# tayloraswift/jpeg

Hardware: AMD Instinct MI355X
Metric: Mpixels/s decode (IDCT+dequant+upsample+YCbCr->RGB); % HBM roofline (higher is better)
Workload: dtype f32; 1 GPU; C3: one 8192x8192 ycc8 4:2:0 image per GPU per step, fused Spectral->RGB8 decode (ring of 4 distinct images); sampling=4:2:0, output=RGB8, coefficients=distribution N (SURVEY 8d), seeded, quanta=CompressionLevel luminance/chrominance(1.0), parallelism=independent images x1 (weak scaling), no data-path collective

## Files before the change

include/jpeg_amd.h:

```cpp
#ifndef JPEG_AMD_H
#define JPEG_AMD_H

#include <stddef.h>
#include <stdint.h>

#ifdef __cplusplus
extern "C" {
#endif

#define JPEG_AMD_VERSION 100
#define JPEG_AMD_MAX_PLANES 4

typedef enum jpeg_amd_status {
    JPEG_AMD_OK      = 0,
    JPEG_AMD_EINVAL  = -1,
    JPEG_AMD_ENOMEM  = -2,
    JPEG_AMD_EHIP    = -3,
    JPEG_AMD_ENODEV  = -4,
    JPEG_AMD_ENOSUP  = -5
} jpeg_amd_status;

typedef struct jpeg_amd_ctx jpeg_amd_ctx;

typedef struct jpeg_amd_layout {
// ... 9 lines not shown
} jpeg_amd_layout;

typedef enum jpeg_amd_color {
    JPEG_AMD_COLOR_YCC8 = 0,
    JPEG_AMD_COLOR_RGB8 = 1
} jpeg_amd_color;

int         jpeg_amd_version(void);
const char *jpeg_amd_strerror(int status);
int         jpeg_amd_device_count(int *count);
#define JPEG_AMD_CTX_OWN_STREAM 1
int         jpeg_amd_ctx_create(int device, void *stream, int flags, jpeg_amd_ctx **ctx);
int         jpeg_amd_ctx_destroy(jpeg_amd_ctx *ctx);
int         jpeg_amd_ctx_synchronize(jpeg_amd_ctx *ctx);
int         jpeg_amd_last_hip_error(const jpeg_amd_ctx *ctx);
int         jpeg_amd_layout_units(jpeg_amd_layout *layout);

int jpeg_amd_malloc(jpeg_amd_ctx *ctx, size_t bytes, void **d_ptr);
int jpeg_amd_free(jpeg_amd_ctx *ctx, void *d_ptr);
int jpeg_amd_memcpy_h2d(jpeg_amd_ctx *ctx, void *d_dst, const void *h_src, size_t bytes);
int jpeg_amd_memcpy_d2h(jpeg_amd_ctx *ctx, void *h_dst, const void *d_src, size_t bytes);
int jpeg_amd_timer_begin(jpeg_amd_ctx *ctx);
int jpeg_amd_timer_end(jpeg_amd_ctx *ctx, float *elapsed_ms);


int jpeg_amd_idct_plane(jpeg_amd_ctx *ctx, const int16_t *d_coef, int units_x, int units_y,
                        const uint16_t h_quanta_zigzag[64], int precision,
                        uint16_t *d_plane);

int jpeg_amd_spectral_idct(jpeg_amd_ctx *ctx, const jpeg_amd_layout *layout,
// ... 257 lines not shown
```

include/jpeg_amd.hpp:

```cpp
#pragma once

#include <cstdint>
#include <algorithm>
#include <array>
#include <map>
#include <memory>
#include <stdexcept>
#include <string>
#include <utility>
#include <vector>

#include "jpeg_amd.h"

namespace jpeg_amd {

struct error : std::runtime_error {
    int status;
    error(int s, const std::string &what) : std::runtime_error(what + ": " + jpeg_amd_strerror(s)), status(s) {}
};
inline void check(int status, const char *what)
{
    if (status != JPEG_AMD_OK) throw error(status, what);
}

class context {
  public:
    explicit context(int device = 0, void *stream = nullptr, bool own_stream = true)
    {
        check(jpeg_amd_ctx_create(device, stream, own_stream ? JPEG_AMD_CTX_OWN_STREAM : 0, &ctx_), "jpeg_amd_ctx_create");
    }
    ~context() { jpeg_amd_ctx_destroy(ctx_); }
    context(const context &) = delete;
    context &operator=(const context &) = delete;
    jpeg_amd_ctx *handle() const { return ctx_; }
    void synchronize() const { check(jpeg_amd_ctx_synchronize(ctx_), "jpeg_amd_ctx_synchronize"); }

  private:
    jpeg_amd_ctx *ctx_ = nullptr;
};

template <class T>
class device_array {
  public:
    device_array() = default;
    device_array(const context &c, size_t n) : ctx_(&c), n_(n)
    {
        void *p = nullptr;
        check(jpeg_amd_malloc(c.handle(), n * sizeof(T), &p), "jpeg_amd_malloc");
        p_ = static_cast<T *>(p);
    }
// ... 360 lines not shown
```

jpeg_amd/_lib.py:

```python
from __future__ import annotations

import ctypes as C
import os

HERE = os.path.dirname(os.path.abspath(__file__))
LIB_PATH = os.environ.get("JPEG_AMD_LIBRARY") or os.path.join(HERE, "libjpeg_amd.so")
MAX_PLANES = 4

OK, EINVAL, ENOMEM, EHIP, ENODEV, ENOSUP = 0, -1, -2, -3, -4, -5
COLOR_YCC8, COLOR_RGB8 = 0, 1
CTX_OWN_STREAM = 1


class JpegAmdError(RuntimeError):
    def __init__(self, status: int, what: str, hip: int = 0):
        self.status, self.hip = status, hip
        msg = lib().jpeg_amd_strerror(status).decode()
        super().__init__(f"{what}: {msg} (status {status}" + (f", hipError {hip})" if hip else ")"))


class Layout(C.Structure):
    _fields_ = [
        ("width", C.c_int32), ("height", C.c_int32), ("precision", C.c_int32),
        ("nplanes", C.c_int32), ("scale_x", C.c_int32), ("scale_y", C.c_int32),
# ... 4 lines not shown


_p = C.c_void_p
_pp = C.POINTER(C.c_void_p)
_szp = C.POINTER(C.c_size_t)
_L = C.POINTER(Layout)

SIGNATURES = {
    "jpeg_amd_version": (C.c_int, []),
    "jpeg_amd_strerror": (C.c_char_p, [C.c_int]),
    "jpeg_amd_device_count": (C.c_int, [C.POINTER(C.c_int)]),
    "jpeg_amd_ctx_create": (C.c_int, [C.c_int, _p, C.c_int, _pp]),
    "jpeg_amd_ctx_destroy": (C.c_int, [_p]),
    "jpeg_amd_ctx_synchronize": (C.c_int, [_p]),
    "jpeg_amd_last_hip_error": (C.c_int, [_p]),
    "jpeg_amd_layout_units": (C.c_int, [_L]),
    "jpeg_amd_malloc": (C.c_int, [_p, C.c_size_t, _pp]),
    "jpeg_amd_free": (C.c_int, [_p, _p]),
    "jpeg_amd_memcpy_h2d": (C.c_int, [_p, _p, _p, C.c_size_t]),
    "jpeg_amd_memcpy_d2h": (C.c_int, [_p, _p, _p, C.c_size_t]),
    "jpeg_amd_timer_begin": (C.c_int, [_p]),
    "jpeg_amd_timer_end": (C.c_int, [_p, C.POINTER(C.c_float)]),
    "jpeg_amd_idct_plane": (C.c_int, [_p, _p, C.c_int, C.c_int, _p, C.c_int, _p]),
    "jpeg_amd_spectral_idct": (C.c_int, [_p, _L, _pp, _p, C.c_int, _pp]),
    "jpeg_amd_planar_interleaved": (C.c_int, [_p, _L, _pp, C.c_int, _p]),
    "jpeg_amd_rectangular_unpack": (C.c_int, [_p, _p, C.c_size_t, C.c_int, C.c_int, _p]),
    "jpeg_amd_decode_batch": (C.c_int, [_p, _L, C.c_int, _pp, _szp, _p, C.c_size_t, C.c_int,
                                        C.c_int, C.c_int, _p, C.c_size_t]),
    "jpeg_amd_decode": (C.c_int, [_p, _L, _pp, _p, C.c_int, C.c_int, C.c_int, _p]),
    "jpeg_amd_spectral_rectangular_batch": (C.c_int, [_p, _L, C.c_int, _pp, _szp, _p, C.c_size_t, C.c_int, C.c_int, _p, C.c_size_t]),
# ... 138 lines not shown
```

jpeg_amd/api.py:

```python
from __future__ import annotations

import ctypes as C
from dataclasses import dataclass
from typing import Dict, List, Optional, Sequence, Tuple

import numpy as np

from . import _lib

MAX_PLANES = _lib.MAX_PLANES


class YCbCr:
    code = _lib.COLOR_YCC8


class RGB:
    code = _lib.COLOR_RGB8


def _torch():
    import torch
    return torch

# ... 8 lines not shown
        self.device = int(device)
        self.torch_device = torch.device("cuda", self.device)
        if stream is None:
            stream = torch.cuda.current_stream(self.torch_device).cuda_stream
        self._h = C.c_void_p()
        flags = _lib.CTX_OWN_STREAM if own_stream else 0
        _lib.check(_lib.lib().jpeg_amd_ctx_create(self.device, C.c_void_p(stream), flags,
                                                 C.byref(self._h)), "jpeg_amd_ctx_create")

    @property
    def handle(self):
        return self._h

    def synchronize(self):
        _lib.check(_lib.lib().jpeg_amd_ctx_synchronize(self._h), "synchronize", self._h)

    def timer_begin(self):
        _lib.check(_lib.lib().jpeg_amd_timer_begin(self._h), "timer_begin", self._h)

    def timer_end(self) -> float:
        ms = C.c_float()
        _lib.check(_lib.lib().jpeg_amd_timer_end(self._h, C.byref(ms)), "timer_end", self._h)
        return ms.value

    def empty(self, n: int, dtype):
        torch = _torch()
        return torch.empty(max(int(n), 0), dtype=dtype, device=self.torch_device)

    def upload(self, a: np.ndarray):
        torch = _torch()
# ... 700 lines not shown
```

jpeg_amd/csrc/capi.hip:

```cpp
#pragma clang fp contract(off)

#include <hip/hip_runtime.h>

#include <cstdio>
#include <cstdlib>
#include <cstring>
#include <new>
#include <algorithm>
#include <atomic>
#include <memory>
#include <chrono>
#include <system_error>
#include <thread>
#include <vector>

#include "interleave.hpp"
#include "kernels.hpp"
#include "transform.hpp"
#include "worker_pool.hpp"

using namespace jpeg_amd;

struct jpeg_amd_ctx {
    int device = 0;
    hipStream_t stream = nullptr;
    bool own_stream = false;
    hipEvent_t ev_begin = nullptr, ev_end = nullptr;
    void *scratch = nullptr;
    size_t scratch_bytes = 0;
    uint16_t *d_qstage = nullptr;
    uint32_t *d_walk = nullptr;
    int32_t *d_flag = nullptr;
    void *d_region = nullptr;
    size_t region_bytes = 0;
    int qslot = 0;
    int last_hip = 0;
    void *file_pinned[2] = {nullptr, nullptr};
    void *file_device = nullptr;
    size_t file_pinned_bytes = 0, file_device_bytes = 0;
    hipEvent_t file_done[2] = {nullptr, nullptr};
    hipEvent_t file_decoded[2] = {nullptr, nullptr};
    hipEvent_t file_fetched[2] = {nullptr, nullptr};
    hipStream_t file_d2h = nullptr;
    std::unique_ptr<WorkerPool> workers, copiers;
    std::vector<std::vector<uint32_t>> records;
};
// ... 380 lines not shown
    if (ctx->ev_end) (void)hipEventDestroy(ctx->ev_end);
    if (ctx->own_stream && ctx->stream) (void)hipStreamDestroy(ctx->stream);
    delete ctx;
    return JPEG_AMD_OK;
}

int jpeg_amd_ctx_synchronize(jpeg_amd_ctx *ctx)
{
    JA_TRY(bind(ctx));
    JA_HIP(ctx, hipStreamSynchronize(ctx->stream));
    return JPEG_AMD_OK;
}

int jpeg_amd_last_hip_error(const jpeg_amd_ctx *ctx) { return ctx ? ctx->last_hip : 0; }

int jpeg_amd_layout_units(jpeg_amd_layout *L)
{
    if (!L || L->nplanes < 1 || L->nplanes > JPEG_AMD_MAX_PLANES || L->scale_x < 1 ||
        L->scale_y < 1 || L->width <= 0 || L->height <= 0)
        return JPEG_AMD_EINVAL;
    for (int p = 0; p < L->nplanes; ++p) {
        if (L->factor_x[p] < 1 || L->factor_y[p] < 1) return JPEG_AMD_EINVAL;
        L->units_x[p] = units_of(L->width * L->factor_x[p], 8 * L->scale_x);
        L->units_y[p] = units_of(L->height * L->factor_y[p], 8 * L->scale_y);
    }
    return JPEG_AMD_OK;
}


int jpeg_amd_malloc(jpeg_amd_ctx *ctx, size_t bytes, void **d_ptr)
// ... 126 lines not shown
                          const uint16_t *d_quanta, size_t quanta_stride, int ntables,
                          int cosited, jpeg_amd_color color, uint8_t *d_pixels,
                          size_t pixel_stride)
{
    JA_TRY(bind(ctx));
    JA_TRY(check_layout(L, ntables));
    JA_TRY(check_planes_cover_image(L));
    JA_TRY(check_batch8(L, n_images, color));
    if (n_images == 0) return JPEG_AMD_OK;
    if (!d_coef || !coef_stride || !d_quanta || !d_pixels) return JPEG_AMD_EINVAL;
    PlaneSet cs;
    JA_TRY(plane_set(L, d_coef, coef_stride, true, &cs));
    const QuantaRef q{d_quanta, quanta_stride};
    const bool rgb = color == JPEG_AMD_COLOR_RGB8;
    if (fused_decode_supported(*L, cosited != 0)) {
        JA_HIP(ctx, launch_fused_decode(ctx->stream, n_images, *L, cs, q, rgb, ctx->d_walk, d_pixels, pixel_stride));
        return JPEG_AMD_OK;
    }
    return staged_decode(ctx, L, n_images, cs, q, cosited != 0, true, rgb ? PixelKind::RGB8 : PixelKind::YCC8, d_pixels, pixel_stride);
}

int jpeg_amd_decode(jpeg_amd_ctx *ctx, const jpeg_amd_layout *L, const int16_t *const d_coef[],
                    const uint16_t *h_quanta, int ntables, int cosited, jpeg_amd_color color,
                    uint8_t *d_pixels)
{
    JA_TRY(bind(ctx));
    JA_TRY(check_layout(L, ntables));
    const uint16_t *d_q = nullptr;
    JA_TRY(stage_quanta(ctx, h_quanta, ntables, &d_q));
    const size_t zero[JPEG_AMD_MAX_PLANES] = {0, 0, 0, 0};
    return jpeg_amd_decode_batch(ctx, L, 1, d_coef, zero, d_q, 0, ntables, cosited, color,
// ... 1333 lines not shown
```

jpeg_amd/csrc/kernels.hpp:

```cpp
#pragma once

#include <hip/hip_runtime.h>
#include <stddef.h>
#include <stdint.h>

#include "../../include/jpeg_amd.h"

namespace jpeg_amd {

typedef uint32_t u32x4_t __attribute__((ext_vector_type(4)));
__device__ __forceinline__ void store_nt16(void *p, const uint4 &v)
{
    __builtin_nontemporal_store(u32x4_t{v.x, v.y, v.z, v.w}, reinterpret_cast<u32x4_t *>(p));
}

struct PlaneSet {
    const void *ptr[JPEG_AMD_MAX_PLANES];
    size_t      stride[JPEG_AMD_MAX_PLANES];
};
struct PlaneSetMut {
    void  *ptr[JPEG_AMD_MAX_PLANES];
    size_t stride[JPEG_AMD_MAX_PLANES];
};

// ... 19 lines not shown
hipError_t launch_planar_to_pixels(hipStream_t stream, int n_images,
                                   const jpeg_amd_layout &layout, const PlaneSet &planes,
                                   bool planes_u8, bool cosited, PixelKind kind,
                                   void *d_out, size_t out_stride_bytes);

bool       generic_encode_supported(const jpeg_amd_layout &layout);
hipError_t launch_generic_encode(hipStream_t stream, int n_images, const jpeg_amd_layout &layout, const uint16_t *d_rect,
                                 size_t rect_stride, QuantaRef q, const PlaneSetMut &coef);

hipError_t launch_unpack(hipStream_t stream, const uint16_t *d_rect, size_t npixels,
                         int nplanes, jpeg_amd_color color, uint8_t *d_pixels);

bool       fused_decode_supported(const jpeg_amd_layout &layout, bool cosited);
hipError_t launch_fused_decode(hipStream_t stream, int n_images, const jpeg_amd_layout &layout,
                               const PlaneSet &coef, QuantaRef q, bool rgb, uint32_t *d_walk_counters,
                               uint8_t *d_pixels, size_t pixel_stride);

bool       quad_decode_supported(const jpeg_amd_layout &layout);
hipError_t launch_quad_decode(hipStream_t stream, int n_images, const jpeg_amd_layout &layout,
                              const PlaneSet &coef, QuantaRef q, bool rgb, uint32_t *d_walk_counters,
                              uint8_t *d_pixels, size_t pixel_stride);

bool       generic_fused_supported(const jpeg_amd_layout &layout);
hipError_t launch_generic_fused(hipStream_t stream, int n_images, const jpeg_amd_layout &layout, const PlaneSet &coef,
                                QuantaRef q, bool cosited, uint32_t *d_walk_counter, uint16_t *d_rect, size_t rect_stride);

uint32_t   region_tiles(const jpeg_amd_region &region);
hipError_t launch_region_decode(hipStream_t stream, int n_images, const jpeg_amd_layout &layout, const PlaneSet &coef, QuantaRef q,
                                bool rgb, const uint32_t *d_tiles, const int32_t *d_regions, uint32_t nwg,
                                uint8_t *d_pixels, size_t pixel_stride);
hipError_t launch_region_crop(hipStream_t stream, int n_images, const uint8_t *d_full, size_t full_stride, int width,
                              const int32_t *d_regions, size_t max_bytes, uint8_t *d_pixels, size_t pixel_stride);

hipError_t launch_scaled_decode(hipStream_t stream, int n_images, const jpeg_amd_layout &layout, int n, int width, int height,
                                const PlaneSet &coef, QuantaRef q, bool rgb, uint8_t *d_pixels, size_t pixel_stride);
hipError_t launch_idct_scaled_plane(hipStream_t stream, int n_images, const int16_t *d_coef, size_t coef_stride, QuantaRef q,
// ... 24 lines not shown
```

jpeg_amd/csrc/kernels_fused.hip:

```cpp
#pragma clang fp contract(off)

#include "dct.hpp"
#include "fused_common.hpp"
#include "kernels.hpp"
#include "upsample.hpp"

#include <algorithm>
#include <cstdlib>

namespace jpeg_amd {

namespace {


struct LumaArgs {
    const int16_t *coef;
    size_t coef_stride;
    const int16_t *ccoef[2];
    size_t ccoef_stride[2];
    int cqi[2];
    const uint16_t *quanta;
    size_t quanta_stride;
    int qi;
    int ux, uy;
// ... 547 lines not shown
    for (int p = 0; p < L.nplanes; ++p) {
        if (L.units_x[p] != units(L.width * L.factor_x[p], 8 * L.scale_x)) return false;
        if (L.units_y[p] != units(L.height * L.factor_y[p], 8 * L.scale_y)) return false;
    }
    if (L.nplanes == 1) return true;
    if (L.nplanes != 3 || cosited) return false;
    if (L.factor_x[0] != L.scale_x || L.factor_y[0] != L.scale_y) return false;
    if (L.scale_x > 2 || L.scale_y > 2) return false;
    for (int p = 1; p < 3; ++p)
        if (L.factor_x[p] != 1 || L.factor_y[p] != 1) return false;
    return true;
}

hipError_t launch_fused_decode(hipStream_t stream, int n_images, const jpeg_amd_layout &L,
                               const PlaneSet &coef, QuantaRef q, bool rgb, uint32_t *d_walk_counters,
                               uint8_t *d_pixels, size_t pixel_stride)
{
    const bool chroma = L.nplanes == 3;
    if (chroma && L.scale_x == 2 && L.scale_y == 2)
        return launch_quad_decode(stream, n_images, L, coef, q, rgb, d_walk_counters, d_pixels, pixel_stride);
    LumaArgs la{};
    if (chroma) {
        for (int i = 0; i < 2; ++i) {
            la.ccoef[i] = static_cast<const int16_t *>(coef.ptr[1 + i]);
            la.ccoef_stride[i] = coef.stride[1 + i];
            la.cqi[i] = L.qi[1 + i];
        }
        la.pw_c = 8 * L.units_x[1]; la.ph_c = 8 * L.units_y[1];
    }
    la.coef = static_cast<const int16_t *>(coef.ptr[0]);
    la.coef_stride = coef.stride[0];
    la.quanta = q.d_quanta; la.quanta_stride = q.image_stride; la.qi = L.qi[0];
    la.ux = L.units_x[0]; la.uy = L.units_y[0];
    la.W = L.width; la.H = L.height;
    la.out = d_pixels; la.out_stride = pixel_stride;
// ... 28 lines not shown
```

jpeg_amd/csrc/kernels_quad.hip:

```cpp
#pragma clang fp contract(off)

#include "dct.hpp"
#include "fused_common.hpp"
#include "kernels.hpp"
#include "upsample.hpp"

#include <algorithm>
#include <cstdlib>

namespace jpeg_amd {

namespace {

JA_PHASE_STORAGE

struct QuadArgs {
    const int16_t *coef[3];
    size_t coef_stride[3];
    const uint16_t *quanta;
    size_t quanta_stride;
    int qi[3];
    int ux, uy;
    int uxc, uyc;
    int W, H;
    uint8_t *out;
    size_t out_stride;
    int tiles_x;
    int sx0;
    uint32_t *tickets;
    int stacks_per_image;
    int nstacks;
};

#ifndef JA_QUAD_WAVES
#define JA_QUAD_WAVES 3
#endif
template <int BX> struct QuadShape {
    static constexpr int BY = 64 / BX;
    static constexpr int QS = kThreads / 64;
};

template <int MODE, int BX, bool FAST, bool DYN>
__global__ __launch_bounds__(kThreads, JA_QUAD_WAVES) void k_quad420(QuadArgs a)
{
    constexpr int BY = QuadShape<BX>::BY, QS = QuadShape<BX>::QS;
    constexpr int NW = kThreads / 64;
    static_assert(QS == 4 && NW == 4, "the roles below are dealt to four waves");
    constexpr int CW = BX * 4, CR = BY * 4;
    constexpr int CBW = BX / 2, CBR = BY / 2;
    constexpr int PITCH = CW / 4 + 2;
    constexpr int QROWS = QS * CR + 2;
    constexpr int PLANE = QROWS * PITCH;
    constexpr int SEG_DW = BX * 6;
    constexpr int CPS = SEG_DW / 4;
    constexpr int NHROW = 4 * CBW, NSIDE = 4 * (QS * CBR + 2);
    constexpr int NDMA_C = 8;

#ifdef JA_X_LDSHACK
    __shared__ __attribute__((aligned(16))) uint32_t coefbuf[NW / 2][64 * 32];
// ... 26 lines not shown
        uint32_t rem, col;
        img = (int)fd_spi.div((uint32_t)q, rem);
        syi = QS * (int)fd_tx.div(rem, col) + qp;
        sxi = (int)col + a.sx0;
    };
    const int strips_y = (a.uy + BY - 1) / BY;
#ifdef JA_X_ROLEROT
    auto role_of = [&](int t) -> int { return (qp + t) & 3; };
#else
    auto role_of = [&](int t) -> int { return (qp + 2 * (t & 1)) & 3; };
#endif

    auto lane_chunk = [&](int lane) -> uint32_t {
        const uint32_t l3 = lane >> 3;
        return l3 * 128 + (((lane & 7) ^ (l3 >> 1)) << 4);
    };
    auto sgpr = [](uint32_t v) -> uint32_t { asm volatile("" : "+s"(v)); return v; };
    auto dma_luma = [&](int img, int syi, int sxi, int lane) {
        const uint32_t ve = lane_chunk(lane);
        const uint32_t ux = sgpr((uint32_t)a.ux);
        const uint32_t row0 = (uint32_t)(BY * syi), rows = (uint32_t)min(BY, a.uy - BY * syi);
        const char *base = reinterpret_cast<const char *>(a.coef[0] + img * a.coef_stride[0]) + ((uint64_t)(row0 * ux) << 7);
        const i32x4_t srd = make_srd(base, (rows * ux) << 7);
#pragma unroll
        for (int r = 0; r < BY; ++r)
            lds_dma16_brun<BX / 8, true>(srd, ((uint32_t)r * ux + (uint32_t)(sxi * BX)) << 7, ve, ve ^ 64u, coef_lds + r * (BX * 128));
    };
    auto dma_chroma = [&](int img, int syi, int sxi, int lane, int role) {
        const int top = syi - qp;
        const uint32_t uxc = sgpr((uint32_t)a.uxc);
// ... 24 lines not shown
            return;
        }
#pragma unroll
        for (int i = 0; i < NDMA_C; ++i) {
            if (8 * i >= NSIDE) break;
            const int b = 8 * i + (lane >> 3);
            const int pl = (b >> 1) & 1, row = min(max(CBR * top - 1 + (b >> 2), 0), a.uyc - 1);
            const int bx = (b & 1) ? CBW * sxi + CBW : CBW * sxi - 1;
            const int16_t *cbase = a.coef[1 + pl] + img * a.coef_stride[1 + pl];
            const uint32_t blk = (bx >= 0 && bx < a.uxc) ? (uint32_t)row * a.uxc + bx : 0u;
            const int c = (lane & 7) ^ ((b >> 1) & 7);
            lds_dma16_keep(reinterpret_cast<const char *>(cbase) + ((size_t)blk * 128 + 16 * c), coef_lds + 1024 * i);
        }
    };

#ifdef JA_X_STAGGER
    for (int d = (int)(blockIdx.x / 256u) * (JA_X_STAGGER); d > 0; d -= 64 * 100) __builtin_amdgcn_s_sleep(100);
#endif
    if ((int)blockIdx.x >= a.nstacks) return;
    constexpr bool dyn = DYN;
    int cur = (int)blockIdx.x;
    const int last_round = a.nstacks - (int)gridDim.x, second_last_round = a.nstacks - 2 * (int)gridDim.x;
    int c_img, c_syi, c_sxi;
    locate(cur, c_img, c_syi, c_sxi);
    dma_chroma(c_img, c_syi, c_sxi, lane0, role_of(0));
    int img_of_table = -1;
    int stores_behind_dma = 0;
    JA_PHASE_DECL

    for (int trip = 0;; ++trip) {
        int lane = lane0;
        asm volatile("" : "+v"(lane));
        const int lbx = lane & (BX - 1), seg = (int)((unsigned)lane / BX);
        const int img = c_img, syi = c_syi, sxi = c_sxi;
        const bool phantom = syi >= strips_y;

        const int table_id = a.quanta_stride == 0 ? 0 : img;
        if (table_id != img_of_table) {
            const int qk = lane & 7, qh = lane >> 3;
#pragma unroll
            for (int p = 0; p < 3; ++p)
                sqw[qp][p][8 * qk + qh] = modulate_entry(qk, qh, 0.125f, a.quanta[img * a.quanta_stride + 64 * a.qi[p] + zigzag_of(qk, qh)]);
            img_of_table = table_id;
        }

        if (stores_behind_dma == 16) asm volatile("s_waitcnt vmcnt(16)" ::: "memory");
        else asm volatile("s_waitcnt vmcnt(0)" ::: "memory");
        JA_PHASE(0)
        __builtin_amdgcn_s_setprio(3);
        uint32_t ticket = 0;
        if (dyn && qp == 0 && lane0 == 0) ticket = __hip_atomic_fetch_add(a.tickets, 1u, __ATOMIC_RELAXED, __HIP_MEMORY_SCOPE_AGENT);
        uint32_t w[32];
        auto read_block = [&]() {
            const uint4 *cw = reinterpret_cast<const uint4 *>(coef_w) + 8 * lane;
            const int sw = (lane >> 1) & 7;
#pragma unroll
            for (int i = 0; i < 8; ++i) {
                const uint4 v = cw[i ^ sw];
                w[4 * i + 0] = v.x; w[4 * i + 1] = v.y; w[4 * i + 2] = v.z; w[4 * i + 3] = v.w;
            }
        };
        read_block();
        const uint32_t done_seen = lds_peek(done);
        asm volatile("s_waitcnt lgkmcnt(0)" ::: "memory");
        if (!phantom) dma_luma(img, syi, sxi, lane);
        __builtin_amdgcn_sched_barrier(0);
        JA_PHASE(1)

        const int top = syi - qp;
        const bool stack_above = top > 0, stack_below = CBR * (top + QS) < a.uyc;
        const bool has_left = sxi > 0, has_right = CBW * sxi + CBW < a.uxc;
        const int first_bad = (a.uxc << 1) - sxi * (CW / 4) + 1;
        auto fix_columns = [&](uint32_t *row) {
            if (!has_left) row[0] = (row[1] & 0xffu) * 0x01010101u;
            if (first_bad < PITCH) {
                const uint32_t last = (row[first_bad - 1] >> 24) * 0x01010101u;
                for (int c = first_bad; c < PITCH; ++c) row[c] = last;
            }
        };
        {
// ... 61 lines not shown
#pragma unroll
                        for (int y = 0; y < 8; ++y) col[(1 + 8 * (rowi - 1) + y) * PITCH] = e[y];
                    }
                }
            }
        }
        lds_arrive(ready);
        JA_PHASE(4)
        if (cur < second_last_round) __builtin_amdgcn_s_setprio(2);
        else if (cur < last_round) __builtin_amdgcn_s_setprio(1);
        else __builtin_amdgcn_s_setprio(0);
        bool more = false;
        auto take = [&](int next) {
            more = next < a.nstacks;
            if (more) {
                int n_img, n_syi, n_sxi;
                locate(next, n_img, n_syi, n_sxi); c_img = n_img; c_syi = n_syi; c_sxi = n_sxi;
                dma_chroma(n_img, n_syi, n_sxi, lane, role_of(trip + 1));
                cur = next;
            }
        };
        auto drawn = [&]() -> int {
            lds_wait_ge(pub, (uint32_t)(trip + 1));
            return __builtin_amdgcn_readfirstlane((int)*(volatile uint32_t *)&next_slot[trip & 1]);
        };
        if (phantom) {
            if (dyn) take(drawn());
            else take(cur + (int)gridDim.x);
            lds_arrive(done);
            stores_behind_dma = 0;
            if (!more) break;
            continue;
        }
// ... 57 lines not shown
        auto finish = [&](float v) -> float {
            return __builtin_fmaf(v, 0.0625f, kMagic - 32768.0f - (MODE == 1 ? 128.0f : 0.0f)) - kMagic;
        };
        float hw[2][3][8];
        uint32_t rawn[2][3];
#pragma unroll
        for (int pl = 0; pl < 2; ++pl) {
            uint32_t r0[3], r1[3];
            hraw(pl, 0, r0); hraw(pl, 1, r1); hraw(pl, 2, rawn[pl]);
            hconv(r0, hw[pl][0]); hconv(r1, hw[pl][1]);
        }

        const int tile_px = min(BX * 8, a.W - BX * 8 * sxi);
        const int nb = 3 * tile_px;
        const uint32_t pitch = 3u * a.W;
        uint8_t *strip_out = a.out + img * a.out_stride + ((size_t)(8 * BY * syi) * a.W + BX * 8 * sxi) * 3;
        int sg0, sg1;
        if constexpr (BX == 32) { sg0 = 1 + ((lane - 48) >> 31); sg1 = 1; }
        else { sg0 = (int)((unsigned)lane / CPS); sg1 = (int)((64u + (unsigned)lane) / CPS); }
        const int j0 = lane - CPS * sg0, j1 = 64 + lane - CPS * sg1;
        const int in0 = 16 * j0 - nb, in1 = max(16 * j1 - nb, lane - 32);
        const bool col0 = in0 < 0, col1 = in1 < 0;
        const int rows_here = min(8 * BY, a.H - 8 * BY * syi);
        const uint32_t strip_bytes = (uint32_t)rows_here * pitch;
        const i32x4_t out_srd = make_srd(strip_out, strip_bytes);
        const int rem0 = col0 ? nb - 16 * j0 : 0, rem1 = col1 ? nb - 16 * j1 : 0;
        const uint32_t base0 = sg0 * 8u * pitch + 16u * j0, base1 = sg1 * 8u * pitch + 16u * j1;
        auto place = [](uint32_t base, int d) -> uint32_t {
            const uint32_t m = (uint32_t)(d >> 31);
            return (base & m) | (0x80000000u & ~m);
        };
        const uint32_t voff0 = place(base0, FAST ? in0 : in0 + 15), voff1 = place(base1, FAST ? in1 : max(16 * j1 - nb + 15, lane - 32));
        stores_behind_dma = FAST ? 16 : 0;
        JA_PHASE(7)

        uint4 pv0 = make_uint4(0, 0, 0, 0), pv1 = make_uint4(0, 0, 0, 0);
        auto store_tail = [&](const uint4 &v, uint32_t base, int rem, uint32_t soff) {
            const __amdgpu_buffer_rsrc_t rsrc = __builtin_amdgcn_make_buffer_rsrc(strip_out, 0, (int)strip_bytes, 0x00020000);
            const bool part = rem > 0 && rem < 16;
            const int nd = rem >> 2, nbytes = rem & 3;
            const uint32_t d[4] = {v.x, v.y, v.z, v.w};
#pragma unroll
            for (int k = 0; k < 3; ++k)
                __builtin_amdgcn_raw_buffer_store_b32(d[k], rsrc, (part && k < nd) ? base + 4u * k : 0x80000000u, soff, 0);
            const uint32_t w = nd == 0 ? v.x : nd == 1 ? v.y : nd == 2 ? v.z : v.w;
#pragma unroll
            for (int b = 0; b < 3; ++b)
// ... 60 lines not shown
            pv1 = *reinterpret_cast<const uint4 *>(stage_w + 4 * (64 + (lane & 31)));
            if ((y & 1) == 1 && y < 7) {
#pragma unroll
                for (int pl = 0; pl < 2; ++pl) hraw(pl, (y >> 1) + 3, rawn[pl]);
                if (y == 5) lds_arrive(done);
            }
        }
        __builtin_amdgcn_sched_barrier(0);
        store_row(7);
        JA_PHASE(10)
        if (!more) break;
    }
    JA_PHASE_FLUSH((int)blockIdx.x * NW + qp, lane0)
}

template <int MODE, int BX, bool FAST, bool DYN>
int quad_resident_workgroups()
{
    return resident_workgroups_of<k_quad420<MODE, BX, FAST, DYN>>(2);
}

template <int MODE, int BX, bool FAST, bool DYN>
hipError_t launch_quad_walk(hipStream_t stream, const QuadArgs &a)
{
    int cap = quad_resident_workgroups<MODE, BX, FAST, DYN>();
#ifdef JA_X_GRID_PER_CU
    cap = std::min(cap, (JA_X_GRID_PER_CU) * (cap / 3));
#endif
#ifdef JA_PHASE_PROFILE
    if (const char *e = std::getenv("JA_GRID_CAP")) cap = std::min(cap, std::atoi(e));
#endif
    hipLaunchKernelGGL((k_quad420<MODE, BX, FAST, DYN>), dim3(std::min(a.nstacks, cap)), dim3(kThreads), 0, stream, a);
    return hipGetLastError();
}
template <int MODE, int BX, bool FAST>
hipError_t launch_quad(hipStream_t stream, const QuadArgs &a)
{
    return a.tickets ? launch_quad_walk<MODE, BX, FAST, true>(stream, a) : launch_quad_walk<MODE, BX, FAST, false>(stream, a);
}

}

#ifdef JA_PHASE_PROFILE
extern "C" int jpeg_amd_debug_phase_cycles(unsigned long long *h_out, size_t n)
{
    return (int)hipMemcpyFromSymbol(h_out, HIP_SYMBOL(g_phase_cycles), n * sizeof(unsigned long long));
}
extern "C" int jpeg_amd_debug_wave_info(unsigned long long *h_out, size_t n)
{
    return (int)hipMemcpyFromSymbol(h_out, HIP_SYMBOL(g_wave_info), n * sizeof(unsigned long long));
}
#endif

// ... 13 lines not shown
#ifdef JA_X_FORCE_BX
    return QuadCut{1, {JA_X_FORCE_BX, 0}, {0, 0}, {(ux + JA_X_FORCE_BX - 1) / JA_X_FORCE_BX, 0}};
#endif
    const long wide = quad_stacks((ux + 31) / 32, uy, 2), narrow = quad_stacks((ux + 15) / 16, uy, 4);
    QuadCut best = narrow < wide ? QuadCut{1, {16, 0}, {0, 0}, {(ux + 15) / 16, 0}} : QuadCut{1, {32, 0}, {0, 0}, {(ux + 31) / 32, 0}};
    const int whole = ux / 32, rest = ux - 32 * whole;
    if (whole > 0 && rest > 0 && rest <= 16) {
        const long mixed = quad_stacks(whole, uy, 2) + quad_stacks(1, uy, 4);
        if (mixed < std::min(wide, narrow) && n_images * std::min(wide, narrow) >= 16 * resident)
            best = QuadCut{2, {32, 16}, {0, 2 * whole}, {whole, 1}};
    }
    return best;
}

hipError_t launch_quad_decode(hipStream_t stream, int n_images, const jpeg_amd_layout &L, const PlaneSet &coef, QuantaRef q,
                              bool rgb, uint32_t *d_walk_counters, uint8_t *d_pixels, size_t pixel_stride)
{
    QuadArgs a{};
    for (int p = 0; p < 3; ++p) {
        a.coef[p] = static_cast<const int16_t *>(coef.ptr[p]);
        a.coef_stride[p] = coef.stride[p];
        a.qi[p] = L.qi[p];
    }
    a.quanta = q.d_quanta; a.quanta_stride = q.image_stride;
    a.ux = L.units_x[0]; a.uy = L.units_y[0];
    a.uxc = L.units_x[1]; a.uyc = L.units_y[1];
    a.W = L.width; a.H = L.height;
    a.out = d_pixels; a.out_stride = pixel_stride;
    if (n_images == 0 || a.ux == 0 || a.uy == 0) return hipSuccess;
    const bool fast = (L.width & 15) == 0 && (pixel_stride & 15) == 0 && (reinterpret_cast<uintptr_t>(d_pixels) & 15) == 0;
    auto resident = [&](int bx) -> int {
// ... 7 lines not shown
        const int bx = cut.bx[part];
        a.tiles_x = cut.cols[part]; a.sx0 = cut.sx0[part];
        a.stacks_per_image = (int)quad_stacks(a.tiles_x, a.uy, 64 / bx);
        const long nstacks = (long)a.stacks_per_image * n_images;
        if (nstacks > 0x3fffffffL) return hipErrorInvalidValue;
        a.nstacks = (int)nstacks;
#ifndef JA_X_TICKET_TRIPS
#define JA_X_TICKET_TRIPS 16
#endif
        a.tickets = nstacks >= (long)(JA_X_TICKET_TRIPS) * resident(bx) ? d_walk_counters : nullptr;
        if (a.tickets) {
            const hipError_t m = hipMemsetAsync(a.tickets, 0, sizeof(uint32_t), stream);
            if (m != hipSuccess) return m;
        }
        hipError_t e;
        if (bx == 16) e = fast ? (rgb ? launch_quad<1, 16, true>(stream, a) : launch_quad<0, 16, true>(stream, a))
                               : (rgb ? launch_quad<1, 16, false>(stream, a) : launch_quad<0, 16, false>(stream, a));
        else e = fast ? (rgb ? launch_quad<1, 32, true>(stream, a) : launch_quad<0, 32, true>(stream, a))
                      : (rgb ? launch_quad<1, 32, false>(stream, a) : launch_quad<0, 32, false>(stream, a));
        if (e != hipSuccess) return e;
    }
    return hipSuccess;
}

}
```

Baseline: 906,100 Mpixels/s.

## Add column-stable static walk variant for single-image quad 4:2:0 decode

Adds a STABLE template variant of the quad 4:2:0 kernel for launches with one image, no tickets, and a grid that divides evenly by tile columns. Each workgroup keeps a fixed tile column and walks down rows with precomputed pointer steps. This avoids recomputing locate(), per-lane chunk offsets and base addresses every trip. It also replaces an env-var grid cap with a context-level grid_cap API. The risk is more register pressure from state carried across trips, and the path only applies when the grid divides evenly by the tile columns.

```diff
diff --git a/include/jpeg_amd.h b/include/jpeg_amd.h
--- a/include/jpeg_amd.h
+++ b/include/jpeg_amd.h
@@ -47,6 +47,7 @@
 int         jpeg_amd_ctx_destroy(jpeg_amd_ctx *ctx);
 int         jpeg_amd_ctx_synchronize(jpeg_amd_ctx *ctx);
 int         jpeg_amd_last_hip_error(const jpeg_amd_ctx *ctx);
+int         jpeg_amd_ctx_set_grid_cap(jpeg_amd_ctx *ctx, int max_workgroups);
 int         jpeg_amd_layout_units(jpeg_amd_layout *layout);
 
 int jpeg_amd_malloc(jpeg_amd_ctx *ctx, size_t bytes, void **d_ptr);
diff --git a/include/jpeg_amd.hpp b/include/jpeg_amd.hpp
--- a/include/jpeg_amd.hpp
+++ b/include/jpeg_amd.hpp
@@ -34,6 +34,7 @@
     context &operator=(const context &) = delete;
     jpeg_amd_ctx *handle() const { return ctx_; }
     void synchronize() const { check(jpeg_amd_ctx_synchronize(ctx_), "jpeg_amd_ctx_synchronize"); }
+    void set_grid_cap(int n) const { check(jpeg_amd_ctx_set_grid_cap(ctx_, n), "jpeg_amd_ctx_set_grid_cap"); }
 
   private:
     jpeg_amd_ctx *ctx_ = nullptr;
diff --git a/jpeg_amd/_lib.py b/jpeg_amd/_lib.py
--- a/jpeg_amd/_lib.py
+++ b/jpeg_amd/_lib.py
@@ -42,6 +42,7 @@
     "jpeg_amd_ctx_destroy": (C.c_int, [_p]),
     "jpeg_amd_ctx_synchronize": (C.c_int, [_p]),
     "jpeg_amd_last_hip_error": (C.c_int, [_p]),
+    "jpeg_amd_ctx_set_grid_cap": (C.c_int, [_p, C.c_int]),
     "jpeg_amd_layout_units": (C.c_int, [_L]),
     "jpeg_amd_malloc": (C.c_int, [_p, C.c_size_t, _pp]),
     "jpeg_amd_free": (C.c_int, [_p, _p]),
diff --git a/jpeg_amd/api.py b/jpeg_amd/api.py
--- a/jpeg_amd/api.py
+++ b/jpeg_amd/api.py
@@ -46,6 +46,9 @@
 
     def synchronize(self):
         _lib.check(_lib.lib().jpeg_amd_ctx_synchronize(self._h), "synchronize", self._h)
+
+    def set_grid_cap(self, max_workgroups: int):
+        _lib.check(_lib.lib().jpeg_amd_ctx_set_grid_cap(self._h, int(max_workgroups)), "set_grid_cap", self._h)
 
     def timer_begin(self):
         _lib.check(_lib.lib().jpeg_amd_timer_begin(self._h), "timer_begin", self._h)
diff --git a/jpeg_amd/csrc/capi.hip b/jpeg_amd/csrc/capi.hip
--- a/jpeg_amd/csrc/capi.hip
+++ b/jpeg_amd/csrc/capi.hip
@@ -30,6 +30,7 @@
     size_t scratch_bytes = 0;
     uint16_t *d_qstage = nullptr;
     uint32_t *d_walk = nullptr;
+    int grid_cap = 0;
     int32_t *d_flag = nullptr;
     void *d_region = nullptr;
     size_t region_bytes = 0;
@@ -440,6 +441,13 @@
 
 int jpeg_amd_last_hip_error(const jpeg_amd_ctx *ctx) { return ctx ? ctx->last_hip : 0; }
 
+int jpeg_amd_ctx_set_grid_cap(jpeg_amd_ctx *ctx, int max_workgroups)
+{
+    if (!ctx || max_workgroups < 0) return JPEG_AMD_EINVAL;
+    ctx->grid_cap = max_workgroups;
+    return JPEG_AMD_OK;
+}
+
 int jpeg_amd_layout_units(jpeg_amd_layout *L)
 {
     if (!L || L->nplanes < 1 || L->nplanes > JPEG_AMD_MAX_PLANES || L->scale_x < 1 ||
@@ -596,7 +604,7 @@
     const QuantaRef q{d_quanta, quanta_stride};
     const bool rgb = color == JPEG_AMD_COLOR_RGB8;
     if (fused_decode_supported(*L, cosited != 0)) {
-        JA_HIP(ctx, launch_fused_decode(ctx->stream, n_images, *L, cs, q, rgb, ctx->d_walk, d_pixels, pixel_stride));
+        JA_HIP(ctx, launch_fused_decode(ctx->stream, n_images, *L, cs, q, rgb, ctx->d_walk, d_pixels, pixel_stride, ctx->grid_cap));
         return JPEG_AMD_OK;
     }
     return staged_decode(ctx, L, n_images, cs, q, cosited != 0, true, rgb ? PixelKind::RGB8 : PixelKind::YCC8, d_pixels, pixel_stride);
diff --git a/jpeg_amd/csrc/kernels.hpp b/jpeg_amd/csrc/kernels.hpp
--- a/jpeg_amd/csrc/kernels.hpp
+++ b/jpeg_amd/csrc/kernels.hpp
@@ -57,12 +57,12 @@
 bool       fused_decode_supported(const jpeg_amd_layout &layout, bool cosited);
 hipError_t launch_fused_decode(hipStream_t stream, int n_images, const jpeg_amd_layout &layout,
                                const PlaneSet &coef, QuantaRef q, bool rgb, uint32_t *d_walk_counters,
-                               uint8_t *d_pixels, size_t pixel_stride);
+                               uint8_t *d_pixels, size_t pixel_stride, int grid_cap = 0);
 
 bool       quad_decode_supported(const jpeg_amd_layout &layout);
 hipError_t launch_quad_decode(hipStream_t stream, int n_images, const jpeg_amd_layout &layout,
                               const PlaneSet &coef, QuantaRef q, bool rgb, uint32_t *d_walk_counters,
-                              uint8_t *d_pixels, size_t pixel_stride);
+                              uint8_t *d_pixels, size_t pixel_stride, int grid_cap = 0);
 
 bool       generic_fused_supported(const jpeg_amd_layout &layout);
 hipError_t launch_generic_fused(hipStream_t stream, int n_images, const jpeg_amd_layout &layout, const PlaneSet &coef,
diff --git a/jpeg_amd/csrc/kernels_fused.hip b/jpeg_amd/csrc/kernels_fused.hip
--- a/jpeg_amd/csrc/kernels_fused.hip
+++ b/jpeg_amd/csrc/kernels_fused.hip
@@ -585,11 +585,11 @@
 
 hipError_t launch_fused_decode(hipStream_t stream, int n_images, const jpeg_amd_layout &L,
                                const PlaneSet &coef, QuantaRef q, bool rgb, uint32_t *d_walk_counters,
-                               uint8_t *d_pixels, size_t pixel_stride)
+                               uint8_t *d_pixels, size_t pixel_stride, int grid_cap)
 {
     const bool chroma = L.nplanes == 3;
     if (chroma && L.scale_x == 2 && L.scale_y == 2)
-        return launch_quad_decode(stream, n_images, L, coef, q, rgb, d_walk_counters, d_pixels, pixel_stride);
+        return launch_quad_decode(stream, n_images, L, coef, q, rgb, d_walk_counters, d_pixels, pixel_stride, grid_cap);
     LumaArgs la{};
     if (chroma) {
         for (int i = 0; i < 2; ++i) {
diff --git a/jpeg_amd/csrc/kernels_quad.hip b/jpeg_amd/csrc/kernels_quad.hip
--- a/jpeg_amd/csrc/kernels_quad.hip
+++ b/jpeg_amd/csrc/kernels_quad.hip
@@ -6,7 +6,6 @@
 #include "upsample.hpp"
 
 #include <algorithm>
-#include <cstdlib>
 
 namespace jpeg_amd {
 
@@ -30,6 +29,9 @@
     uint32_t *tickets;
     int stacks_per_image;
     int nstacks;
+    int trip_rows;
+    uint32_t chroma_step;
+    size_t luma_step, out_step;
 };
 
 #ifndef JA_QUAD_WAVES
@@ -40,9 +42,10 @@
     static constexpr int QS = kThreads / 64;
 };
 
-template <int MODE, int BX, bool FAST, bool DYN>
+template <int MODE, int BX, bool FAST, bool DYN, bool STABLE = false>
 __global__ __launch_bounds__(kThreads, JA_QUAD_WAVES) void k_quad420(QuadArgs a)
 {
+    static_assert(!(DYN && STABLE), "the column-stable variant is a static walk");
     constexpr int BY = QuadShape<BX>::BY, QS = QuadShape<BX>::QS;
     constexpr int NW = kThreads / 64;
     static_assert(QS == 4 && NW == 4, "the roles below are dealt to four waves");
@@ -99,6 +102,24 @@
     auto lane_chunk = [&](int lane) -> uint32_t {
         const uint32_t l3 = lane >> 3;
         return l3 * 128 + (((lane & 7) ^ (l3 >> 1)) << 4);
+    };
+    struct Chunks { uint32_t base0, base1, voff0, voff1; int rem0, rem1; };
+    auto chunks_of = [](int lane, int nb, uint32_t pitch) -> Chunks {
+        int sg0, sg1;
+        if constexpr (BX == 32) { sg0 = 1 + ((lane - 48) >> 31); sg1 = 1; }
+        else { sg0 = (int)((unsigned)lane / CPS); sg1 = (int)((64u + (unsigned)lane) / CPS); }
+        const int j0 = lane - CPS * sg0, j1 = 64 + lane - CPS * sg1;
+        const int in0 = 16 * j0 - nb, in1 = max(16 * j1 - nb, lane - 32);
+        const bool col0 = in0 < 0, col1 = in1 < 0;
+        Chunks c;
+        c.rem0 = col0 ? nb - 16 * j0 : 0; c.rem1 = col1 ? nb - 16 * j1 : 0;
+        c.base0 = sg0 * 8u * pitch + 16u * j0; c.base1 = sg1 * 8u * pitch + 16u * j1;
+        auto place = [](uint32_t base, int d) -> uint32_t {
+            const uint32_t m = (uint32_t)(d >> 31);
+            return (base & m) | (0x80000000u & ~m);
+        };
+        c.voff0 = place(c.base0, FAST ? in0 : in0 + 15); c.voff1 = place(c.base1, FAST ? in1 : max(16 * j1 - nb + 15, lane - 32));
+        return c;
     };
     auto sgpr = [](uint32_t v) -> uint32_t { asm volatile("" : "+s"(v)); return v; };
     auto dma_luma = [&](int img, int syi, int sxi, int lane) {
@@ -153,6 +174,58 @@
         }
     };
 
+    [[maybe_unused]] uint32_t st_ve = 0, st_voff0 = 0, st_voff1 = 0;
+    [[maybe_unused]] const char *st_side = nullptr;
+    [[maybe_unused]] uint32_t st_side_rb = 0, st_side_c = 0;
+    [[maybe_unused]] uint64_t st_lbase = 0, st_obase = 0;
+    [[maybe_unused]] uint32_t st_ctop = 0;
+    [[maybe_unused]] auto dma_luma_st = [&](int syi, int sxi) {
+        const uint32_t coef_lds_s = sgpr(coef_lds);
+        const uint32_t rb = sgpr((uint32_t)a.ux << 7), col = (uint32_t)(sxi * BX) << 7;
+        const uint32_t rows = (uint32_t)min(BY, a.uy - BY * syi);
+        const i32x4_t srd = make_srd(reinterpret_cast<const char *>(st_lbase), rows * rb);
+#pragma unroll
+        for (int r = 0; r < BY; ++r)
+            lds_dma16_brun<BX / 8, true>(srd, col + (uint32_t)r * rb, st_ve, st_ve ^ 64u, coef_lds_s + r * (BX * 128));
+    };
+    [[maybe_unused]] auto dma_chroma_st = [&](int lane, int role, int syi) {
+        const uint32_t rb = sgpr((uint32_t)a.uxc << 7), at = st_ctop, coef_lds_s = sgpr(coef_lds);
+        auto off = [&](int k) -> uint32_t { return at + (uint32_t)k * rb; };
+        if (role < 3) {
+            const uint32_t ve = st_ve;
+            const uint32_t plane_bytes = (uint32_t)a.uyc * rb;
+            const i32x4_t srd_b = make_srd(reinterpret_cast<const char *>(a.coef[1]), plane_bytes);
+            const i32x4_t srd_r = make_srd(reinterpret_cast<const char *>(a.coef[2]), plane_bytes);
+            if constexpr (BX == 32) {
+#pragma unroll
+                for (int u = 0; u < 4; ++u) {
+                    const uint32_t o = role < 2 ? off(2 * role + (u >> 1)) : ((u >> 1) ? off(CBR * QS) : off(-1));
+                    lds_dma16_brun<2, false>((u & 1) ? srd_r : srd_b, o, ve, ve ^ 64u, coef_lds_s + 2048 * u);
+                }
+            } else if (role < 2) {
+#pragma unroll
+                for (int i = 0; i < NDMA_C; ++i)
+                    lds_dma16_brun<1, false>(((i >> 1) & 1) ? srd_r : srd_b, off(CBR * (2 * role + (i >> 2)) + (i & 1)),
+                                             (i & 1) ? ve ^ 64u : ve, 0u, coef_lds_s + 1024 * i);
+            } else {
+#pragma unroll
+                for (int i = 0; i < NHROW / 8; ++i)
+                    lds_dma16_brun<1, false>((i & 1) ? srd_r : srd_b, (i >> 1) ? off(CBR * QS) : off(-1),
+                                             (i & 1) ? ve ^ 64u : ve, 0u, coef_lds_s + 1024 * i);
+            }
+        } else {
+            const int sub = lane >> 5, last = a.uyc - 1, row0 = CBR * (syi - qp) - 1;
+            const uint32_t c_odd = st_side_c ^ 64u;
+#pragma unroll
+            for (int i = 0; i < NDMA_C; ++i) {
+                if (8 * i >= NSIDE) break;
+                const int row = min(max(row0 + 2 * i + sub, 0), last);
+                lds_dma16_keep(st_side + (__umul24((uint32_t)row, st_side_rb) + ((i & 1) ? c_odd : st_side_c)), coef_lds_s + 1024 * i);
+            }
+        }
+        st_ctop += a.chroma_step;
+    };
+
 #ifdef JA_X_STAGGER
     for (int d = (int)(blockIdx.x / 256u) * (JA_X_STAGGER); d > 0; d -= 64 * 100) __builtin_amdgcn_s_sleep(100);
 #endif
@@ -162,7 +235,27 @@
     const int last_round = a.nstacks - (int)gridDim.x, second_last_round = a.nstacks - 2 * (int)gridDim.x;
     int c_img, c_syi, c_sxi;
     locate(cur, c_img, c_syi, c_sxi);
-    dma_chroma(c_img, c_syi, c_sxi, lane0, role_of(0));
+    if constexpr (STABLE) {
+        const int sxi = c_sxi, top = c_syi - qp;
+        st_ve = lane_chunk(lane0);
+        const uint32_t pitch = 3u * a.W;
+        const Chunks ck = chunks_of(lane0, 3 * min(BX * 8, a.W - BX * 8 * sxi), pitch);
+        st_voff0 = ck.voff0; st_voff1 = ck.voff1;
+        {
+            const int l3 = lane0 >> 3, pl = (l3 >> 1) & 1, c = (lane0 & 7) ^ (l3 >> 1);
+            const int bx = (l3 & 1) ? CBW * sxi + CBW : CBW * sxi - 1;
+            const bool inside = bx >= 0 && bx < a.uxc;
+            st_side = reinterpret_cast<const char *>(a.coef[1 + pl]) + ((inside ? (size_t)bx * 128 : 0) + 16 * (c & 3));
+            st_side_rb = inside ? (uint32_t)a.uxc << 7 : 0u;
+            st_side_c = (uint32_t)(c & 4) << 4;
+        }
+        st_ctop = sgpr(((uint32_t)(CBR * top) * (uint32_t)a.uxc + (uint32_t)(CBW * sxi)) << 7);
+        st_lbase = reinterpret_cast<uint64_t>(a.coef[0]) + ((uint64_t)((uint32_t)(BY * c_syi) * (uint32_t)a.ux) << 7) - a.luma_step;
+        st_obase = reinterpret_cast<uint64_t>(a.out) + ((size_t)(8 * BY * c_syi) * a.W + BX * 8 * sxi) * 3 - a.out_step;
+        dma_chroma_st(lane0, role_of(0), c_syi);
+    } else {
+        dma_chroma(c_img, c_syi, c_sxi, lane0, role_of(0));
+    }
     int img_of_table = -1;
     int stores_behind_dma = 0;
     JA_PHASE_DECL
@@ -171,7 +264,8 @@
         int lane = lane0;
         asm volatile("" : "+v"(lane));
         const int lbx = lane & (BX - 1), seg = (int)((unsigned)lane / BX);
-        const int img = c_img, syi = c_syi, sxi = c_sxi;
+        const int img = STABLE ? 0 : c_img, syi = c_syi, sxi = c_sxi;
+        if constexpr (STABLE) { st_lbase += a.luma_step; st_obase += a.out_step; }
         const bool phantom = syi >= strips_y;
 
         const int table_id = a.quanta_stride == 0 ? 0 : img;
@@ -202,7 +296,10 @@
         read_block();
         const uint32_t done_seen = lds_peek(done);
         asm volatile("s_waitcnt lgkmcnt(0)" ::: "memory");
-        if (!phantom) dma_luma(img, syi, sxi, lane);
+        if (!phantom) {
+            if constexpr (STABLE) dma_luma_st(syi, sxi);
+            else dma_luma(img, syi, sxi, lane);
+        }
         __builtin_amdgcn_sched_barrier(0);
         JA_PHASE(1)
 
@@ -294,9 +391,14 @@
         auto take = [&](int next) {
             more = next < a.nstacks;
             if (more) {
-                int n_img, n_syi, n_sxi;
-                locate(next, n_img, n_syi, n_sxi); c_img = n_img; c_syi = n_syi; c_sxi = n_sxi;
-                dma_chroma(n_img, n_syi, n_sxi, lane, role_of(trip + 1));
+                if constexpr (STABLE) {
+                    c_syi += QS * a.trip_rows;
+                    dma_chroma_st(lane, role_of(trip + 1), c_syi);
+                } else {
+                    int n_img, n_syi, n_sxi;
+                    locate(next, n_img, n_syi, n_sxi); c_img = n_img; c_syi = n_syi; c_sxi = n_sxi;
+                    dma_chroma(n_img, n_syi, n_sxi, lane, role_of(trip + 1));
+                }
                 cur = next;
             }
         };
@@ -384,23 +486,15 @@
         const int tile_px = min(BX * 8, a.W - BX * 8 * sxi);
         const int nb = 3 * tile_px;
         const uint32_t pitch = 3u * a.W;
-        uint8_t *strip_out = a.out + img * a.out_stride + ((size_t)(8 * BY * syi) * a.W + BX * 8 * sxi) * 3;
-        int sg0, sg1;
-        if constexpr (BX == 32) { sg0 = 1 + ((lane - 48) >> 31); sg1 = 1; }
-        else { sg0 = (int)((unsigned)lane / CPS); sg1 = (int)((64u + (unsigned)lane) / CPS); }
-        const int j0 = lane - CPS * sg0, j1 = 64 + lane - CPS * sg1;
-        const int in0 = 16 * j0 - nb, in1 = max(16 * j1 - nb, lane - 32);
-        const bool col0 = in0 < 0, col1 = in1 < 0;
+        uint8_t *strip_out = STABLE ? reinterpret_cast<uint8_t *>(st_obase)
+                                    : a.out + img * a.out_stride + ((size_t)(8 * BY * syi) * a.W + BX * 8 * sxi) * 3;
+        const Chunks ck = chunks_of(lane, nb, pitch);
+        const int rem0 = ck.rem0, rem1 = ck.rem1;
+        const uint32_t base0 = ck.base0, base1 = ck.base1;
         const int rows_here = min(8 * BY, a.H - 8 * BY * syi);
         const uint32_t strip_bytes = (uint32_t)rows_here * pitch;
         const i32x4_t out_srd = make_srd(strip_out, strip_bytes);
-        const int rem0 = col0 ? nb - 16 * j0 : 0, rem1 = col1 ? nb - 16 * j1 : 0;
-        const uint32_t base0 = sg0 * 8u * pitch + 16u * j0, base1 = sg1 * 8u * pitch + 16u * j1;
-        auto place = [](uint32_t base, int d) -> uint32_t {
-            const uint32_t m = (uint32_t)(d >> 31);
-            return (base & m) | (0x80000000u & ~m);
-        };
-        const uint32_t voff0 = place(base0, FAST ? in0 : in0 + 15), voff1 = place(base1, FAST ? in1 : max(16 * j1 - nb + 15, lane - 32));
+        const uint32_t voff0 = STABLE ? st_voff0 : ck.voff0, voff1 = STABLE ? st_voff1 : ck.voff1;
         stores_behind_dma = FAST ? 16 : 0;
         JA_PHASE(7)
 
@@ -491,29 +585,45 @@
     JA_PHASE_FLUSH((int)blockIdx.x * NW + qp, lane0)
 }
 
-template <int MODE, int BX, bool FAST, bool DYN>
+template <int MODE, int BX, bool FAST, bool DYN, bool STABLE = false>
 int quad_resident_workgroups()
 {
-    return resident_workgroups_of<k_quad420<MODE, BX, FAST, DYN>>(2);
-}
-
-template <int MODE, int BX, bool FAST, bool DYN>
-hipError_t launch_quad_walk(hipStream_t stream, const QuadArgs &a)
-{
-    int cap = quad_resident_workgroups<MODE, BX, FAST, DYN>();
+    return resident_workgroups_of<k_quad420<MODE, BX, FAST, DYN, STABLE>>(2);
+}
+
+template <int MODE, int BX, bool FAST, bool DYN, bool STABLE = false>
+int quad_grid(const QuadArgs &a, int grid_cap)
+{
+    int cap = quad_resident_workgroups<MODE, BX, FAST, DYN, STABLE>();
 #ifdef JA_X_GRID_PER_CU
     cap = std::min(cap, (JA_X_GRID_PER_CU) * (cap / 3));
 #endif
-#ifdef JA_PHASE_PROFILE
-    if (const char *e = std::getenv("JA_GRID_CAP")) cap = std::min(cap, std::atoi(e));
-#endif
-    hipLaunchKernelGGL((k_quad420<MODE, BX, FAST, DYN>), dim3(std::min(a.nstacks, cap)), dim3(kThreads), 0, stream, a);
+    if (grid_cap > 0) cap = std::min(cap, grid_cap);
+    return std::min(a.nstacks, cap);
+}
+
+template <int MODE, int BX, bool FAST>
+hipError_t launch_quad(hipStream_t stream, QuadArgs a, int grid_cap)
+{
+    if (a.tickets) {
+        hipLaunchKernelGGL((k_quad420<MODE, BX, FAST, true>), dim3(quad_grid<MODE, BX, FAST, true>(a, grid_cap)), dim3(kThreads), 0, stream, a);
+        return hipGetLastError();
+    }
+    if (a.nstacks == a.stacks_per_image) {
+        const int grid = quad_grid<MODE, BX, FAST, false, true>(a, grid_cap);
+        if (grid % a.tiles_x == 0 && a.nstacks > grid) {
+            constexpr int BY = QuadShape<BX>::BY, QS = QuadShape<BX>::QS;
+            a.trip_rows = grid / a.tiles_x;
+            const size_t strip_rows = (size_t)QS * a.trip_rows;
+            a.chroma_step = (uint32_t)(strip_rows * (BY / 2) * a.uxc) << 7;
+            a.luma_step = (strip_rows * BY * a.ux) << 7;
+            a.out_step = strip_rows * 8 * BY * a.W * 3;
+            hipLaunchKernelGGL((k_quad420<MODE, BX, FAST, false, true>), dim3(grid), dim3(kThreads), 0, stream, a);
+            return hipGetLastError();
+        }
+    }
+    hipLaunchKernelGGL((k_quad420<MODE, BX, FAST, false>), dim3(quad_grid<MODE, BX, FAST, false>(a, grid_cap)), dim3(kThreads), 0, stream, a);
     return hipGetLastError();
-}
-template <int MODE, int BX, bool FAST>
-hipError_t launch_quad(hipStream_t stream, const QuadArgs &a)
-{
-    return a.tickets ? launch_quad_walk<MODE, BX, FAST, true>(stream, a) : launch_quad_walk<MODE, BX, FAST, false>(stream, a);
 }
 
 }
@@ -557,7 +667,7 @@
 }
 
 hipError_t launch_quad_decode(hipStream_t stream, int n_images, const jpeg_amd_layout &L, const PlaneSet &coef, QuantaRef q,
-                              bool rgb, uint32_t *d_walk_counters, uint8_t *d_pixels, size_t pixel_stride)
+                              bool rgb, uint32_t *d_walk_counters, uint8_t *d_pixels, size_t pixel_stride, int grid_cap)
 {
     QuadArgs a{};
     for (int p = 0; p < 3; ++p) {
@@ -595,10 +705,10 @@
             if (m != hipSuccess) return m;
         }
         hipError_t e;
-        if (bx == 16) e = fast ? (rgb ? launch_quad<1, 16, true>(stream, a) : launch_quad<0, 16, true>(stream, a))
-                               : (rgb ? launch_quad<1, 16, false>(stream, a) : launch_quad<0, 16, false>(stream, a));
-        else e = fast ? (rgb ? launch_quad<1, 32, true>(stream, a) : launch_quad<0, 32, true>(stream, a))
-                      : (rgb ? launch_quad<1, 32, false>(stream, a) : launch_quad<0, 32, false>(stream, a));
+        if (bx == 16) e = fast ? (rgb ? launch_quad<1, 16, true>(stream, a, grid_cap) : launch_quad<0, 16, true>(stream, a, grid_cap))
+                               : (rgb ? launch_quad<1, 16, false>(stream, a, grid_cap) : launch_quad<0, 16, false>(stream, a, grid_cap));
+        else e = fast ? (rgb ? launch_quad<1, 32, true>(stream, a, grid_cap) : launch_quad<0, 32, true>(stream, a, grid_cap))
+                      : (rgb ? launch_quad<1, 32, false>(stream, a, grid_cap) : launch_quad<0, 32, false>(stream, a, grid_cap));
         if (e != hipSuccess) return e;
     }
     return hipSuccess;
```

New measurement: 892,200 Mpixels/s. -1.5%, worse.
